# drtconway/zotmer

Measured on AMD Instinct MI355X. Metric: Gk-mers/sec kmerize k=25 on synthetic 150bp FASTQ; achieved HBM GB/s fraction, higher is better.
Workload: dtype u64

## Files before the change

zotmer_amd/csrc/context.hip:

```cpp
#include <stdarg.h>
#include <string.h>

#include "internal.hpp"
#include <vector>

namespace zk {

int fail(zk_ctx* c, int code, const char* fmt, ...) {
    char buf[512];
    va_list ap;
    va_start(ap, fmt);
    vsnprintf(buf, sizeof buf, fmt, ap);
    va_end(ap);
    if (c) c->last_error = buf;
    return code;
}

void arena_reset(zk_ctx* c) { c->arena_off = 0; }

int arena_alloc(zk_ctx* c, uint64_t bytes, void** p) {
    const uint64_t need = (bytes + 255) & ~255ull;
    if (c->arena_off + need > c->arena_size) {
        if (c->arena_off != 0)
            return fail(c, ZK_ENOMEM, "workspace too small: %llu bytes in use, %llu more needed, %llu reserved (call zk_reserve)",
// ... 254 lines not shown
    ZK_TRY(arena_alloc(c, workspace_bytes, &p));
    arena_reset(c);
    return ZK_OK;
}

int zk_release_workspace(zk_ctx* c) {
    if (!c) return ZK_EINVAL;
    enter(c);
    ZK_HIP(c, hipStreamSynchronize(c->stream));
    if (c->arena) { ZK_HIP(c, hipFree(c->arena)); c->arena = nullptr; c->arena_size = 0; c->arena_off = 0; }
    if (c->aux) { ZK_HIP(c, hipFree(c->aux)); c->aux = nullptr; c->aux_size = 0; }
    if (c->status) { ZK_HIP(c, hipFree(c->status)); c->status = nullptr; c->status_words = 0; c->epoch = 0; }
    if (c->part16) { ZK_HIP(c, hipFree(c->part16)); c->part16 = nullptr; c->part16_words = 0; }
    return ZK_OK;
}

int zk_mem_info(zk_ctx* c, uint64_t* free_bytes, uint64_t* total_bytes) {
    if (!c) return ZK_EINVAL;
    enter(c);
    size_t f = 0, t = 0;
    ZK_HIP(c, hipMemGetInfo(&f, &t));
    if (free_bytes) *free_bytes = f;
    if (total_bytes) *total_bytes = t;
    return ZK_OK;
}

int zk_tune(zk_ctx* c, int what, int value) {
    if (!c) return ZK_EINVAL;
    enter(c);
    if (what == ZK_TUNE_SORT_VARIANT) { c->sort_variant = value; return ZK_OK; }
    if (what == ZK_TUNE_PAIRS_VARIANT) { c->pairs_variant = value; return ZK_OK; }
    if (what == ZK_TUNE_SHORT_SORT) { c->short_sort = value; return ZK_OK; }
    if (what == ZK_TUNE_SIDE_DIV) { c->side_div = value; return ZK_OK; }
    if (what == ZK_TUNE_WIDE_TILES) { c->wide_tiles = value ? 1 : 0; return ZK_OK; }
    if (what == ZK_TUNE_PACKED_PAIRS) { c->packed_pairs = value ? 1 : 0; return ZK_OK; }
    if (what == ZK_TUNE_EARLY_COLLAPSE) { c->early_collapse = value < 0 ? 0 : (value > 3 ? 3 : value); return ZK_OK; }
    if (what == ZK_TUNE_COMM_SELF_LOOP) { c->comm_self_loop = value ? 1 : 0; return ZK_OK; }
    if (what == ZK_TUNE_COMM_CHUNK) { c->comm_chunk_bytes = value > 0 ? (uint64_t)value : 0; return ZK_OK; }
    if (what == ZK_TUNE_STREAM_PASS) {
#ifdef ZK_PHASES
        c->stream_pass = value < 0 ? 0 : value;
#else
        if (value < 0 || value > 3) return fail(c, ZK_EINVAL, "stream pass variant %d (0, 1, 2 or 3)", value);
        c->stream_pass = value;
#endif
        return ZK_OK;
    }
    if (what == ZK_TUNE_TAG_WORDS) { c->tag_words = value < 0 ? 0 : (value > 2 ? 2 : value); return ZK_OK; }
    if (what == ZK_TUNE_DEDUPE_VARIANT) { c->dedupe_variant = value < 0 ? -1 : (value & 3); return ZK_OK; }
    if (what == ZK_TUNE_KWAY) { c->kway = value < 0 ? 0 : (value > 2 ? 2 : value); return ZK_OK; }
    if (what == ZK_TUNE_TILE_SORT) { c->tile_sort = value ? 1 : 0; return ZK_OK; }
    if (what == ZK_TUNE_TAG_PASS) { c->tag_pass = value ? 1 : 0; return ZK_OK; }
    if (what == ZK_TUNE_DEDUPE_BITS) { c->dedupe_bits = value < 0 ? 0 : value; return ZK_OK; }
    if (what == ZK_TUNE_STRAND_BLOCKS) { c->strand_blocks = value < 0 ? 0 : (value > 5 ? 1 : value); return ZK_OK; }
    if (what == ZK_TUNE_DEDUPE_LIMIT) { c->dedupe_limit = value < 1 ? 1 : (value > 65536 ? 65536 : value); return ZK_OK; }
    if (what == ZK_TUNE_STREAM_RANGES) { c->stream_ranges = value < 0 ? 0 : (value > 4096 ? 4096 : value); return ZK_OK; }
    if (what == ZK_TUNE_XCD_GROUP) {
        if (value < 0 || value > 32 || (value & (value - 1))) return fail(c, ZK_EINVAL, "xcd group must be 0 or a power of two <= 32");
        c->xcd_group = value;
        return ZK_OK;
    }
    return fail(c, ZK_EINVAL, "unknown tuning knob %d", what);
}

int zk_debug_buffer(zk_ctx* c, void* d_buf) {
    if (!c) return ZK_EINVAL;
    enter(c);
    c->dbg = (u64*)d_buf;
    return ZK_OK;
}

int zk_profile(zk_ctx* c, int enable) {
    if (!c) return ZK_EINVAL;
    enter(c);
    ZK_HIP(c, hipStreamSynchronize(c->stream));
    for (auto& r : c->prof) { (void)hipEventDestroy(r.a); (void)hipEventDestroy(r.b); }
    c->prof.clear();
    c->profile = enable != 0;
    return ZK_OK;
}

int zk_profile_read(zk_ctx* c, int tag, uint64_t* launches, double* total_ms, uint64_t* total_bytes) {
    if (!c) return ZK_EINVAL;
    enter(c);
    ZK_HIP(c, hipStreamSynchronize(c->stream));
    uint64_t n = 0, bytes = 0;
    double ms = 0;
    for (auto& r : c->prof) {
        if (r.tag != tag) continue;
        float t = 0;
        ZK_HIP(c, hipEventElapsedTime(&t, r.a, r.b));
        n++; ms += t; bytes += r.bytes;
    }
    if (launches) *launches = n;
    if (total_ms) *total_ms = ms;
    if (total_bytes) *total_bytes = bytes;
    return ZK_OK;
}

int zk_alloc(zk_ctx* c, uint64_t bytes, void** dptr) {
    if (!c || !dptr) return ZK_EINVAL;
    enter(c);
    *dptr = nullptr;
    if (bytes == 0) bytes = 256;
    hipError_t e = hipMalloc(dptr, bytes);
    if (e != hipSuccess) return fail(c, ZK_ENOMEM, "hipMalloc(%llu) failed: %s", (unsigned long long)bytes, hipGetErrorString(e));
    return ZK_OK;
// ... 61 lines not shown
```

zotmer_amd/csrc/internal.hpp:

```cpp
#pragma once
#include <hip/hip_runtime.h>
#include <stddef.h>
#include <stdint.h>
#include <stdio.h>
#include <string>
#include <vector>

#include "../../include/zotk.h"
#include "common.hpp"

struct zk_strand_counters { u32 n_declined, fail; };
struct zk_scalars {
    u64 rle_side;
    u64 total;
    u64 acgt[4];
    u64 n_keys;
    u64 rec_info[3];
    u64 sample_n;
    u64 dedupe_flags, dedupe_n_retry, dedupe_counter, dedupe_n_big, dedupe_n_bad;
    u64 dedupe_m_cursor;
    u64 dedupe_n_in;
    u64 dedupe_n_out;
    zk_strand_counters strand;
    u64 hist_big_n;
// ... 121 lines not shown
            return zk::fail((c), ZK_EHIP, "%s failed: %s (%s:%d)", #call, hipGetErrorString(e__), __FILE__, __LINE__); \
    } while (0)
#define ZK_ARGS(c, cond) do { if (!(c)) return ZK_EINVAL; zk::enter(c); if (!(cond)) return zk::fail((c), ZK_EINVAL, "bad argument: %s", #cond); } while (0)
#define ZK_TRY(expr)             \
    do {                         \
        int r__ = (expr);        \
        if (r__ != ZK_OK) return r__; \
    } while (0)

void arena_reset(zk_ctx* c);
int arena_alloc(zk_ctx* c, uint64_t bytes, void** p);
int arena_require(zk_ctx* c, uint64_t want, uint64_t must);
int aux_require(zk_ctx* c, uint64_t bytes, char** p);
int lookback_begin(zk_ctx* c, uint64_t words, uint32_t tiles, u32* epoch, u32* ticket_base);
int part16_begin(zk_ctx* c, uint64_t words, unsigned short** out);
int check_device_error(zk_ctx* c);

void prof_begin(zk_ctx* c, int tag, uint64_t algorithmic_bytes);
void prof_end(zk_ctx* c);
void prof_add_bytes(zk_ctx* c, int tag, uint64_t bytes);

int fetch_span(zk_ctx* c, void* h_first, size_t bytes, const void* from = nullptr);
template <class T> static inline int fetch(zk_ctx* c, T* h_field, const void* from = nullptr) { return fetch_span(c, h_field, sizeof(T), from); }
int stream_sync(zk_ctx* c);

static inline uint64_t div_up(uint64_t a, uint64_t b) { return (a + b - 1) / b; }
static inline u32 grid_cap(const zk_ctx* c, uint64_t blocks, int per_cu) {
    const uint64_t mx = (uint64_t)c->num_cus * per_cu;
    return (u32)(blocks < mx ? blocks : mx);
}

constexpr int MAX_PASSES = 8;
struct PassPlan {
    int passes;
    int shift[MAX_PASSES];
    int bits[MAX_PASSES];
};
static inline PassPlan make_plan(int key_bits, int rbits, int lo = 0) {
    PassPlan p;
    if (key_bits < 1) key_bits = 1;
    if (key_bits > 64) key_bits = 64;
    p.passes = (key_bits + rbits - 1) / rbits;
    int base = key_bits / p.passes, rem = key_bits % p.passes, s = lo;
    for (int i = 0; i < MAX_PASSES; i++) { p.shift[i] = 0; p.bits[i] = 0; }
    for (int i = 0; i < p.passes; i++) {
        p.bits[i] = base + (i < rem ? 1 : 0);
        p.shift[i] = s;
        s += p.bits[i];
    }
    return p;
}
int sort_keys(zk_ctx* c, u64* keys, u64* alt, uint64_t n, int key_bits, u64** result);
int sort_pairs(zk_ctx* c, u64* keys, u64* alt, u32* vals, u32* valt, uint64_t n, int key_bits, u64** rk, u32** rv);
int sort_keys_upper(zk_ctx* c, u64* keys, u64* alt, uint64_t n, int key_bits, int lo_bit, u64** result, int prof_tag = ZK_PROF_PASS_PACKED);
int sort_pairs_upper(zk_ctx* c, u64* keys, u64* alt, u32* vals, u32* valt, uint64_t n, int key_bits, int lo_bit, u64** rk, u32** rv);
int sort_pairs_mirrored(zk_ctx* c, const u64* src_k, const u32* src_v, u64* keys, u64* alt, u32* vals, u32* valt, uint64_t n, int K,
                        u64** rk, u32** rv, int lo_bit = 0);
int sort_pairs_rbits(zk_ctx* c);
struct StreamSample { int shift; uint64_t value; double max_ratio; uint64_t seen = 0, distinct = 0; bool want_distinct = false; };
struct StreamTags { bool written = false; u64* cuts = nullptr; uint32_t blocks = 0; };
struct StreamSrc { const u8* stream; uint64_t n_bytes; int K; int mode; int lo_bit; int hi_bit = 0; StreamSample* sample = nullptr;
                   StreamTags* tags = nullptr; };
int sort_stream(zk_ctx* c, const StreamSrc& src, u64* buf_a, u64* buf_b, uint64_t cap, uint64_t* n_keys,
                uint64_t acgt[4], u64** result);
int sort_rbits(zk_ctx* c);
PassPlan sort_plan_upper(zk_ctx* c, int key_bits, int lo_bit);
int sort_first_bits(zk_ctx* c, int key_bits, int lo_bit);
constexpr int MIRROR_RBITS = 9, MIRROR_RADIX = 1 << MIRROR_RBITS;
struct MirrorHist { int passes; int shift[4]; int bits[4]; u64* raw; };
int sort_keys_upper_counted(zk_ctx* c, u64* keys, u64* alt, uint64_t n, int key_bits, int lo_bit, u64* counted, u64** result);
struct DedupeMirror { u64* out = nullptr; uint64_t cap = 0; int K = 0; };
struct DedupeResult {
    uint64_t n_out = 0;
    uint32_t flags = 0;
    uint32_t n_big = 0;
    u64 *cuts = nullptr, *nwords = nullptr, *incl = nullptr, *big = nullptr, *work = nullptr;
    u32* sub = nullptr;
    uint32_t chunks = 0;
    int pack = 0;
    int tag_bits = 0;
    bool unsorted = false;
    bool m_emitted = false;
    u64* m_words = nullptr;
    uint64_t m_cap = 0, m_placed = 0;
    MirrorHist mh = {};
    u32* retry = nullptr;
    uint32_t n_retry = 0;
};
int dedupe_pass(zk_ctx* c, const u64* keys, uint64_t n, int key_bits, int b, int pack, u64* work, uint64_t cap, DedupeResult* r,
                uint64_t* n_in = nullptr, uint64_t max_chunks = 0, const u32* tags = nullptr, const u64* tag_cuts = nullptr,
                bool unsorted = false, const DedupeMirror* mirror = nullptr);
int expand_tags(zk_ctx* c, const u32* tags, const u64* cuts, uint32_t blocks, int tag_bits, u64* keys_out, uint64_t first_block = 0, uint64_t n_blocks = 0);
int dedupe_finish(zk_ctx* c, const DedupeResult& r, u64* out_k, u32* out_c, u64* out_m = nullptr, int K = 0, int gbases = 0,
                  u64** mirror_hist = nullptr, int* mirror_group_bits = nullptr, bool packed_out = false);
int dedupe_sort_blocks(zk_ctx* c, DedupeResult& r);
int strand_blocks(zk_ctx* c, const DedupeResult& r, u64* keys_buf, uint64_t buf_words, int K, u64* out_k, u32* out_c, uint64_t cap,
                  uint64_t* n_out);
int collapse_pass(zk_ctx* c, const u64* keys, uint64_t n, int shift, int bits, int pack, u64* out, uint64_t cap, uint64_t* n_out,
                  uint64_t max_tiles = 0);
struct StreamRows { u32* rows = nullptr; u64* offs = nullptr; u32 ranges = 0, radix = 0; u32* gcodes = nullptr; u16* gvalid = nullptr;
                    u32 strands = 1;
                    bool wide = false; };
int stream_hist(zk_ctx* c, const u8* stream, uint64_t n_bytes, int K, int mode, const PassPlan& plan, u64* ghist, u32 gstride,
                u64* d_acgt, u64* d_n, u64* rec_info, u64* sample, u32 sample_cap, int sample_shift, u64 sample_value, u32* sample_n,
                void* image_room, uint64_t image_room_bytes, StreamRows* out);
struct StreamPlanes { u16* dig; int shift, bits; };
int stream_pass0(zk_ctx* c, uint64_t n_bytes, int K, int mode, int shift, int bits, const u64* ghist0, const StreamRows& rows,
                 uint64_t first_nl, bool uniform, u64* kout, uint64_t n, int variant, const StreamPlanes* planes = nullptr);
int stream_pass1(zk_ctx* c, const u32* tags, const u16* dig, uint64_t n, const u64* ghist0, uint32_t radix0, int bits1, u32* tout, u64* cuts);
int tile_sort_top_bits(uint64_t n, int key_bits, int rbits);
int tile_sort(zk_ctx* c, u64* keys, u32* vals, uint64_t n, int key_bits, int top, bool* declined);
int tile_sort_count(zk_ctx* c, const u64* keys, uint64_t n, int key_bits, int top, u64* uniq, u32* counts, uint64_t cap, uint64_t* n_unique,
                    bool* declined);
int trim(zk_ctx* c, const u64* keys, const void* cnts, int cbits, uint64_t n, u64 lo, u64 hi, u64* ok, void* oc,
         uint64_t cap, uint64_t* n_out);
int project_dedupe(zk_ctx* c, const u64* keys, uint64_t n, int shift, u64* out, uint64_t cap, uint64_t* n_out);
int subsample(zk_ctx* c, const u64* keys, uint64_t n, u64 seed, double p, u64* out, uint64_t cap, uint64_t* n_out);
int sample_pairs(zk_ctx* c, const u64* keys, const u64* cnts, uint64_t n, u64 seed, double p, u64* ok, u64* oc, uint64_t cap,
                 uint64_t* n_out);
int subsample_pairs(zk_ctx* c, u64* keys, u32* cnts, uint64_t n, u64 seed, double p, uint64_t* n_out);
int encode_list(zk_ctx* c, const u8* stream, uint64_t n_bytes, int K, int both, u64* out, uint64_t cap, uint64_t* n_out,
                uint64_t acgt[4]);
int capture_filter(zk_ctx* c, const u8* stream, uint64_t n_bytes, int K, const u64* baits, uint64_t n_baits, u8* out,
// ... 38 lines not shown
```

zotmer_amd/csrc/radix_sort.hip:

```cpp
#include <stdlib.h>
#include "internal.hpp"
#include "encode_tile.hpp"

namespace zk {

constexpr int MAX_RADIX = 1024;

enum { SRC_ARRAY = 0, SRC_STREAM = 1 };

template <int BLOCK_, int ITEMS_, int RBITS_, int ROUNDS_ = 1, int WPE_ = 1, int SEG_ = 32, bool PIPE_ = false>
struct Cfg {
    static constexpr int BLOCK = BLOCK_, ITEMS = ITEMS_, RBITS = RBITS_, ROUNDS = ROUNDS_, WPE = WPE_, SEG = SEG_;
    static constexpr bool PIPE = PIPE_;
    static_assert(SEG == 0 || (BLOCK * ITEMS < 32768 && (SEG & (SEG - 1)) == 0), "16-bit tile counts");
    static constexpr int TILE = BLOCK * ITEMS, RADIX = 1 << RBITS, NW = BLOCK / 64;
    static constexpr int EXCH = TILE / ROUNDS, IPR = ITEMS / ROUNDS;
    static_assert(ITEMS % ROUNDS == 0, "ROUNDS");
    static constexpr int DPT = (RADIX + BLOCK - 1) / BLOCK;
    static_assert(ITEMS % 2 == 0 && 2 * ITEMS < 256, "ITEMS");
    static_assert(64 * ITEMS < 65536, "per-wave ranks are 16-bit");
    static_assert(RADIX <= MAX_RADIX && RBITS * MAX_PASSES >= 64, "RBITS");
};

struct SortArgs {
// ... 580 lines not shown
                const u32 s = tid + i * BLOCK;
                if (lo + s < total && gpos[i] < a.n) a.vout[gpos[i]] = exv[s];
            }
        }
    }
#ifdef ZK_STAMPS
    asm volatile("s_waitcnt vmcnt(0)" ::: "memory");
    ZK_STAMP(7);
#endif
}

#ifdef ZK_STAMPS
#define PSTAMP(t, k) do { if (a.dbg && threadIdx.x == 0) a.dbg[(u64)(t) * 8 + (k)] = __builtin_amdgcn_s_memtime(); } while (0)
#define PSTAT(t) ((a.dbg2 && threadIdx.x == 0) ? a.dbg2 + (t) : nullptr)
#else
#define PSTAMP(t, k) do { } while (0)
#define PSTAT(t) nullptr
#endif
__device__ __forceinline__ u32 tile_of(u32 x, u32 k, u32 nx, u32 glog) {
    return ((((k >> glog) * nx) + x) << glog) | (k & ((1u << glog) - 1u));
}
__device__ __forceinline__ u32 steal_tile(const SortArgs& a, u32 x, u32 tiles) {
    for (u32 y = 1; y < a.nx; y++) {
        const u32 xx = (x + y) % a.nx;
        const u32 t = tile_of(xx, atomicAdd(a.xticket + 32 * xx, 1u), a.nx, a.glog);
        if (t < tiles) return t;
    }
    return 0xffffffffu;
}

template <class C, bool PAIRS = false>
struct PipeSmem {
    static constexpr bool IMG_FITS = sizeof(TileImage<C::TILE>) <= sizeof(u16) * C::NW * C::RADIX;
    static constexpr int IMG_WORDS = (int)(sizeof(u16) * C::NW * C::RADIX / 8);
    static constexpr int IMG_T = IMG_FITS ? (IMG_WORDS - 3) * 16 : 16;
    u64 exch[C::TILE];
    u32 exv[PAIRS ? C::TILE : 1];
    union {
        u16 cnt[C::NW][C::RADIX];
        TileImage<PipeSmem::IMG_T> img;
    };
    u32 digit_off[C::RADIX];
    u64 gbase[C::RADIX];
    u32 wsum[C::NW];
    u32 ticket;
    u32 total_live;
    u32 abort;
};

template <class C, int SRC, int VAR = 0>
__global__ __launch_bounds__(C::BLOCK, C::WPE) void pass_pipe_kernel(SortArgs a, u32 tiles) {
    constexpr int BLOCK = C::BLOCK, ITEMS = C::ITEMS, RADIX = C::RADIX, NW = C::NW, DPT = C::DPT, TILE = C::TILE;
    constexpr bool PAIRS = VAR == 5 || VAR == 6;
    constexpr bool ATOM = VAR == 3 || VAR == 4 || VAR == 6, TAGS = VAR == 2 || VAR == 3;
    static_assert(!PAIRS || SRC == SRC_ARRAY, "pairs come from arrays");
    static_assert(!ATOM || (SRC == SRC_ARRAY && NW >= 2), "the counters of the adds are the first two rows of the per-wave counters");
    static_assert(C::ROUNDS == 1, "the pipeline parks a whole tile in LDS");
    constexpr int NS = RADIX / 64;
    __shared__ PipeSmem<C, VAR == 5 || VAR == 6> sm;
    static_assert(SRC == SRC_ARRAY || PipeSmem<C>::IMG_FITS, "the tile image lives in the counter area");
    static_assert(SRC == SRC_ARRAY || (ITEMS == 16 && PipeSmem<C>::IMG_WORDS <= 2 * BLOCK), "stream source: 16 consecutive windows per thread");
    const int tid = threadIdx.x, lane = tid & 63, wave = __builtin_amdgcn_readfirstlane(tid >> 6);
    const u32 dmask = (1u << a.bits) - 1u;
    u16* mycnt = sm.cnt[wave];

    if (tid == 0) sm.abort = 0;
    u32* cnt32 = reinterpret_cast<u32*>(&sm.cnt[0][0]);
    if (ATOM && tid < RADIX) cnt32[tid] = 0;
    bool dirty = false;
    const u32 first = take_ticket(a.ticket, &sm.ticket) - a.ticket_base;
    if (first < (u32)NS) {
        constexpr int U = 32;
        __builtin_amdgcn_s_setprio(3);
        u64* carry = sm.exch;
        if (tid < 64) carry[tid] = 0;
        __syncthreads();
        const u64 tag = st_pack(ZK_ST_INCLUSIVE, a.epoch, 0);
        const u32 batches = (tiles + U - 1) / U;
        for (u32 b = (u32)wave; b < batches; b += NW) {
            const u32 t0 = b * U;
            const u32 nt = (tiles - t0 < (u32)U) ? tiles - t0 : (u32)U;
            __amdgpu_buffer_rsrc_t rs = __builtin_amdgcn_make_buffer_rsrc((void*)(a.part + (u64)t0 * RADIX + (u64)first * 64), 0, 0x7fffffff, 0x00020000);
            __amdgpu_buffer_rsrc_t rd = __builtin_amdgcn_make_buffer_rsrc((void*)(a.status + (u64)t0 * RADIX + (u64)first * 64), 0, 0x7fffffff, 0x00020000);
            u16 x[U];
#pragma unroll
            for (int k = 0; k < U; k++)
                x[k] = ((u32)k < nt) ? (u16)__builtin_amdgcn_raw_buffer_load_b16(rs, 2 * lane, k * RADIX * 2, 16) : (u16)0x8000u;
            for (int spins = 0;; spins++) {
                u32 all = 0x8000u;
#pragma unroll
                for (int k = 0; k < U; k++) all &= x[k];
                if (all & 0x8000u) break;
                if (spins > ZK_SPIN_LIMIT) { atomicOr(a.err, ZK_DERR_SPIN_TIMEOUT | (8u << 8)); break; }
                __builtin_amdgcn_s_sleep(2);
#pragma unroll
                for (int k = 0; k < U; k++)
                    if (!(x[k] & 0x8000u)) x[k] = (u16)__builtin_amdgcn_raw_buffer_load_b16(rs, 2 * lane, k * RADIX * 2, 16);
            }
            u32 sum = 0;
#pragma unroll
            for (int k = 0; k < U; k++) {
                x[k] &= 0x7fffu;
                sum += x[k];
            }
            volatile u64* cw = carry + lane;
            u64 cv = *cw;
            int spins = 0;
// ... 417 lines not shown

    static int begin_pass(zk_ctx* c, SortArgs& a, u32 tiles, u32 tickets, bool pipe, bool stamps = true) {
        const bool seg = !pipe && C::SEG > 0;
        ZK_TRY(lookback_begin(c, seg ? ((uint64_t)tiles / (C::SEG > 0 ? C::SEG : 1) + 2) * C::RADIX : (uint64_t)tiles * C::RADIX, tickets,
                              &a.epoch, &a.ticket_base));
        if (pipe || seg) ZK_TRY(part16_begin(c, (uint64_t)tiles * C::RADIX, &a.part));
        a.status = c->status;
        a.ticket = c->d_ticket;
        a.err = c->d_err;
        a.dbg = stamps ? c->dbg : nullptr;
        a.dbg2 = (stamps && c->dbg) ? c->dbg + 8ull * tiles : nullptr;
        return ZK_OK;
    }
    template <bool PAIRS>
    static int begin_pipe(zk_ctx* c, SortArgs& a, u32 tiles, u32* grid, bool stamps) {
        u32 g = (u32)c->num_cus * (sizeof(PipeSmem<C, PAIRS>) > 80 * 1024 ? 1 : 2);
        if (g > tiles) g = tiles;
        g += C::RADIX / 64;
        ZK_TRY(begin_pass(c, a, tiles, g, true, stamps));
        ZK_HIP(c, hipMemsetAsync(c->d_xticket, 0, 8 * 32 * sizeof(u32), c->stream));
        a.xticket = c->d_xticket;
        a.nx = 1u;
        a.glog = 0;
        *grid = g;
        return ZK_OK;
    }

    template <int SRC, bool PAIRS>
    static int launch_pass(zk_ctx* c, SortArgs a) {
        const u32 tiles = tiles_for(a, SRC);
        if (tiles == 0) return ZK_OK;
        ZK_TRY(begin_pass(c, a, tiles, tiles, false));
        prof_begin(c, SRC == SRC_STREAM ? ZK_PROF_PASS_STREAM : (PAIRS ? ZK_PROF_PASS_PAIRS : ZK_PROF_PASS_KEYS),
                   SRC == SRC_STREAM ? a.n_bytes + 8 * a.n : (PAIRS ? 24 : 16) * a.n);
        hipLaunchKernelGGL((pass_kernel<C, SRC, PAIRS>), dim3(tiles), dim3(C::BLOCK), 0, c->stream, a);
        prof_end(c);
        ZK_HIP(c, hipGetLastError());
        return ZK_OK;
    }

    template <int SRC>
    static int launch_pipe(zk_ctx* c, SortArgs a) {
      if constexpr (C::PIPE) {
        const u32 tiles = tiles_for(a, SRC);
        if (tiles == 0) return ZK_OK;
        u32 grid;
        ZK_TRY(begin_pipe<false>(c, a, tiles, &grid, true));
        a.nx = (c->xcd_group > 0 && c->num_xcd == 8) ? 8u : 1u;
        while ((1 << (a.glog + 1)) <= c->xcd_group) a.glog++;
        prof_begin(c, SRC == SRC_STREAM ? ZK_PROF_PASS_STREAM : (a.prof_tag ? a.prof_tag : ZK_PROF_PASS_KEYS),
                   SRC == SRC_STREAM ? a.n_bytes + 8 * a.n : (a.tags_out ? 12 : 16) * a.n);
        if (SRC == SRC_ARRAY && a.tags_out && a.straddle)
            hipLaunchKernelGGL((pass_pipe_kernel<C, SRC_ARRAY, 3>), dim3(grid), dim3(C::BLOCK), 0, c->stream, a, tiles);
        else if (SRC == SRC_ARRAY && a.straddle)
            hipLaunchKernelGGL((pass_pipe_kernel<C, SRC_ARRAY, 4>), dim3(grid), dim3(C::BLOCK), 0, c->stream, a, tiles);
        else if (SRC == SRC_ARRAY && a.tags_out)
            hipLaunchKernelGGL((pass_pipe_kernel<C, SRC_ARRAY, 2>), dim3(grid), dim3(C::BLOCK), 0, c->stream, a, tiles);
        else if (SRC == SRC_ARRAY && a.prof_tag == ZK_PROF_PASS_PACKED)
            hipLaunchKernelGGL((pass_pipe_kernel<C, SRC, 1>), dim3(grid), dim3(C::BLOCK), 0, c->stream, a, tiles);
        else
            hipLaunchKernelGGL((pass_pipe_kernel<C, SRC, 0>), dim3(grid), dim3(C::BLOCK), 0, c->stream, a, tiles);
        prof_end(c);
        ZK_HIP(c, hipGetLastError());
      }
      return ZK_OK;
    }
    static constexpr bool PIPE_PAIRS = C::PIPE && C::ITEMS <= 8;
    static int launch_pipe_pairs(zk_ctx* c, SortArgs a) {
      if constexpr (PIPE_PAIRS) {
        const u32 tiles = (u32)div_up(a.n, C::TILE);
        if (tiles == 0) return ZK_OK;
        u32 grid;
        ZK_TRY(begin_pipe<true>(c, a, tiles, &grid, false));
        prof_begin(c, ZK_PROF_PASS_PAIRS, 24 * a.n);
        if (a.straddle) hipLaunchKernelGGL((pass_pipe_kernel<C, SRC_ARRAY, 6>), dim3(grid), dim3(C::BLOCK), 0, c->stream, a, tiles);
        else hipLaunchKernelGGL((pass_pipe_kernel<C, SRC_ARRAY, 5>), dim3(grid), dim3(C::BLOCK), 0, c->stream, a, tiles);
        prof_end(c);
        ZK_HIP(c, hipGetLastError());
      }
      return ZK_OK;
    }
    static constexpr bool WIDE = C::PIPE && C::RBITS == 9 && C::BLOCK == 512;
    static u32 keys_pass_tile(zk_ctx* c) { return (WIDE && c->wide_tiles) ? 16384u : (u32)C::TILE; }
    static int launch_keys_pass(zk_ctx* c, const SortArgs& a) {
        if (WIDE && c->wide_tiles) return launch_wide_pass(c, a);
        if (C::PIPE) return launch_pipe<SRC_ARRAY>(c, a);
        return launch_pass<SRC_ARRAY, false>(c, a);
    }

    template <int SRC>
    static int launch_hist(zk_ctx* c, const SortArgs& src, const PassPlan& plan, u64* ghist, u64* acgt, u64* d_n,
                           u64* sample = nullptr, u32 sample_cap = 0, int sample_shift = 0, u64 sample_value = 0) {
        HistArgs h;
        h.sample = sample; h.sample_cap = sample_cap; h.sample_shift = sample_shift; h.sample_value = sample_value;
        h.sample_n = (u32*)&c->d_scalars->sample_n;
        if (sample) ZK_HIP(c, hipMemsetAsync(h.sample_n, 0, sizeof(u64), c->stream));
        h.src = src;
        h.plan = plan;
        h.ghist = ghist;
        h.acgt = acgt;
        h.tiles = tiles_for(src, SRC);
        h.rec_info = nullptr;
        ZK_HIP(c, hipMemsetAsync(ghist, 0, sizeof(u64) * MAX_PASSES * C::RADIX, c->stream));
        if (SRC == SRC_STREAM && src.n_bytes) {
            h.rec_info = c->d_scalars->rec_info;
            ZK_HIP(c, hipMemsetAsync(h.rec_info, 0, 3 * sizeof(u64), c->stream));
            hipLaunchKernelGGL(first_newline_kernel, dim3(1), dim3(256), 0, c->stream, src.stream, (u64)src.n_bytes, h.rec_info);
        }
        if (acgt) ZK_HIP(c, hipMemsetAsync(acgt, 0, sizeof(u64) * 4, c->stream));
        u32 grid = grid_cap(c, h.tiles, 8);
        if (grid == 0) grid = 1;
        prof_begin(c, SRC == SRC_STREAM ? ZK_PROF_HIST_STREAM : ZK_PROF_HIST_ARRAY, SRC == SRC_STREAM ? src.n_bytes : 8 * src.n);
        if constexpr (SRC == SRC_STREAM && C::ITEMS == 16 && C::BLOCK <= 512) {
            if (src.mode != ZK_KEYS_BOTH) hipLaunchKernelGGL((hist_kernel<C, SRC, true>), dim3(grid), dim3(C::BLOCK), 0, c->stream, h);
            else hipLaunchKernelGGL((hist_kernel<C, SRC, false>), dim3(grid), dim3(C::BLOCK), 0, c->stream, h);
        } else {
            hipLaunchKernelGGL((hist_kernel<C, SRC, false>), dim3(grid), dim3(C::BLOCK), 0, c->stream, h);
        }
        prof_end(c);
        ZK_HIP(c, hipGetLastError());
        hipLaunchKernelGGL(hist_scan_kernel, dim3(1), dim3(256), 0, c->stream, ghist, plan.passes, (int)C::RADIX, d_n);
        ZK_HIP(c, hipGetLastError());
        return ZK_OK;
    }

    static int sort_keys(zk_ctx* c, u64* keys, u64* alt, uint64_t n, int key_bits, u64** result, int lo_bit = 0, int prof_tag = 0,
                         u64* counted = nullptr) {
        PassPlan plan = make_plan(key_bits - lo_bit, C::RBITS, lo_bit);
        u64* ghist = counted;
        if (!counted) ZK_TRY(arena_alloc(c, sizeof(u64) * MAX_PASSES * C::RADIX, (void**)&ghist));
        SortArgs a = {};
        a.kin = keys; a.n = n;
        a.prof_tag = prof_tag;
        if (counted) {
            hipLaunchKernelGGL(hist_scan_kernel, dim3(1), dim3(256), 0, c->stream, ghist, plan.passes, (int)C::RADIX, &c->d_scalars->n_keys);
            ZK_HIP(c, hipGetLastError());
        } else {
            ZK_TRY(launch_hist<SRC_ARRAY>(c, a, plan, ghist, nullptr, &c->d_scalars->n_keys));
        }
        u64* in = keys; u64* out = alt;
        for (int p = 0; p < plan.passes; p++) {
            a.kin = in; a.kout = out; a.shift = plan.shift[p]; a.bits = plan.bits[p];
            a.ghist = ghist + p * C::RADIX;
            ZK_TRY(launch_keys_pass(c, a));
            u64* t = in; in = out; out = t;
        }
        *result = in;
        return ZK_OK;
    }

    static int sort_pairs(zk_ctx* c, u64* keys, u64* alt, u32* vals, u32* valt, uint64_t n, int key_bits, u64** rk, u32** rv,
                          const u64* src_k = nullptr, const u32* src_v = nullptr, int mirror_K = 0, int lo_bit = 0, bool unordered = false) {
        PassPlan plan = make_plan(key_bits - lo_bit, C::RBITS, lo_bit);
        u64* ghist;
        ZK_TRY(arena_alloc(c, sizeof(u64) * MAX_PASSES * C::RADIX, (void**)&ghist));
        SortArgs a = {};
        a.kin = mirror_K ? src_k : keys; a.n = n; a.mirror_K = mirror_K;
        ZK_TRY(launch_hist<SRC_ARRAY>(c, a, plan, ghist, nullptr, &c->d_scalars->n_keys));
        const u64* in = mirror_K ? src_k : keys; const u32* vi = mirror_K ? src_v : vals;
        u64* out = mirror_K ? keys : alt; u32* vo = mirror_K ? vals : valt;
        for (int p = 0; p < plan.passes; p++) {
            a.kin = in; a.kout = out; a.vin = vi; a.vout = vo; a.shift = plan.shift[p]; a.bits = plan.bits[p];
            a.ghist = ghist + p * C::RADIX;
            a.mirror_K = (p == 0) ? mirror_K : 0;
            if constexpr (PIPE_PAIRS) {
                a.straddle = nullptr;
                if (unordered && p <= 1)
                    ZK_TRY(straddle_bitmap(c, n, (u32)C::TILE, p == 1 ? ghist : nullptr, 1u << plan.bits[0], (u32)C::RADIX, &a.straddle));
                ZK_TRY(launch_pipe_pairs(c, a));
            } else
            ZK_TRY((launch_pass<SRC_ARRAY, true>(c, a)));
            in = out; vi = vo;
            out = (out == keys) ? alt : keys;
            vo = (vo == vals) ? valt : vals;
        }
        *rk = const_cast<u64*>(in); *rv = const_cast<u32*>(vi);
        return ZK_OK;
    }

    static int stream_count(zk_ctx* c, const StreamSrc& src, const StreamPlan& sp, const SortArgs& a, u64* ghist, u64* buf_b, uint64_t cap,
                            StreamRows* srows, uint64_t* n, uint64_t acgt[4]) {
        u64* d_acgt = c->d_scalars->acgt;
        u64* d_n = &c->d_scalars->n_keys;
        u64* sample = sp.sampling ? buf_b : nullptr;
        const int sample_shift = sp.sampling ? src.sample->shift : 0;
        const u64 sample_value = sp.sampling ? src.sample->value : 0;
        if (sp.ranged) {
            u64* rec_info = c->d_scalars->rec_info;
            ZK_HIP(c, hipMemsetAsync(rec_info, 0, ZK_SPAN(rec_info, sample_n), c->stream));
            hipLaunchKernelGGL(first_newline_kernel, dim3(1), dim3(256), 0, c->stream, src.stream, (u64)src.n_bytes, rec_info);
            ZK_TRY(stream_hist(c, src.stream, src.n_bytes, src.K, src.mode, sp.plan, ghist, (u32)C::RADIX, d_acgt, d_n, rec_info,
                               sample, SAMPLE_CAP, sample_shift, sample_value, (u32*)&c->d_scalars->sample_n,
                               (char*)buf_b + (sp.sampling ? 24ull * SAMPLE_CAP : 0), 8 * cap - (sp.sampling ? 24ull * SAMPLE_CAP : 0), srows));
            hipLaunchKernelGGL(hist_scan_kernel, dim3(1), dim3(256), 0, c->stream, ghist, sp.plan.passes, (int)C::RADIX, d_n);
            ZK_HIP(c, hipGetLastError());
        } else {
// ... 142 lines not shown
typedef Cfg<1024, 8, 9, 1, 4, 32, true> V7;
static_assert(V3::RBITS == MIRROR_RBITS && V3::RADIX == MIRROR_RADIX, "dedupe_finish counts the digits of the default geometry");
int launch_wide_pass(zk_ctx* c, const SortArgs& a) { return Sorter<V6>::launch_pipe<SRC_ARRAY>(c, a); }
#define ZK_SORT_CASES(CALL)                         \
        case 0: return Sorter<V0>::CALL;            \
        case 1: return Sorter<V1>::CALL;            \
        case 2: return Sorter<V2>::CALL;            \
        case 4: return Sorter<V4>::CALL;            \
        case 5: return Sorter<V5>::CALL;            \
        case 6: return Sorter<V6>::CALL;            \
        default: return Sorter<V3>::CALL;
#define ZK_SORT_DISPATCH(c, CALL) switch ((c)->sort_variant) { ZK_SORT_CASES(CALL) }
#define ZK_PAIRS_DISPATCH(c, CALL) switch ((c)->pairs_variant) { case 7: return Sorter<V7>::CALL; ZK_SORT_CASES(CALL) }

static int sort_keys_lsd(zk_ctx* c, u64* keys, u64* alt, uint64_t n, int key_bits, u64** result) {
    ZK_SORT_DISPATCH(c, sort_keys(c, keys, alt, n, key_bits, result));
}
static int sort_pairs_lsd(zk_ctx* c, u64* keys, u64* alt, u32* vals, u32* valt, uint64_t n, int key_bits, u64** rk, u32** rv) {
    ZK_PAIRS_DISPATCH(c, sort_pairs(c, keys, alt, vals, valt, n, key_bits, rk, rv));
}

int sort_keys(zk_ctx* c, u64* keys, u64* alt, uint64_t n, int key_bits, u64** result) {
    *result = keys;
    if (n == 0) return ZK_OK;
    const int top = c->tile_sort ? tile_sort_top_bits(n, key_bits, sort_rbits(c)) : 0;
    if (top) {
        u64* res = nullptr;
        bool declined = false;
        ZK_TRY(sort_keys_upper(c, keys, alt, n, key_bits, key_bits - top, &res, ZK_PROF_PASS_KEYS));
        ZK_TRY(tile_sort(c, res, nullptr, n, key_bits, top, &declined));
        *result = res;
        if (!declined) return ZK_OK;
        return sort_keys_lsd(c, res, res == keys ? alt : keys, n, key_bits, result);
    }
    return sort_keys_lsd(c, keys, alt, n, key_bits, result);
}

int sort_pairs(zk_ctx* c, u64* keys, u64* alt, u32* vals, u32* valt, uint64_t n, int key_bits, u64** rk, u32** rv) {
    *rk = keys; *rv = vals;
    if (n == 0) return ZK_OK;
    const int top = c->tile_sort ? tile_sort_top_bits(n, key_bits, sort_pairs_rbits(c)) : 0;
    if (top) {
        u64* k1 = nullptr; u32* v1 = nullptr;
        bool declined = false;
        ZK_TRY(sort_pairs_upper(c, keys, alt, vals, valt, n, key_bits, key_bits - top, &k1, &v1));
        ZK_TRY(tile_sort(c, k1, v1, n, key_bits, top, &declined));
        *rk = k1; *rv = v1;
        if (!declined) return ZK_OK;
        return sort_pairs_lsd(c, k1, k1 == keys ? alt : keys, v1, v1 == vals ? valt : vals, n, key_bits, rk, rv);
    }
    return sort_pairs_lsd(c, keys, alt, vals, valt, n, key_bits, rk, rv);
}

int sort_keys_upper(zk_ctx* c, u64* keys, u64* alt, uint64_t n, int key_bits, int lo_bit, u64** result, int prof_tag) {
    *result = keys;
    if (n == 0 || lo_bit >= key_bits) return ZK_OK;
    ZK_SORT_DISPATCH(c, sort_keys(c, keys, alt, n, key_bits, result, lo_bit, prof_tag));
}

int sort_keys_upper_counted(zk_ctx* c, u64* keys, u64* alt, uint64_t n, int key_bits, int lo_bit, u64* counted, u64** result) {
    *result = keys;
    if (n == 0 || lo_bit >= key_bits) return ZK_OK;
    return Sorter<V3>::sort_keys(c, keys, alt, n, key_bits, result, lo_bit, ZK_PROF_PASS_PACKED, counted);
}

int sort_pairs_upper(zk_ctx* c, u64* keys, u64* alt, u32* vals, u32* valt, uint64_t n, int key_bits, int lo_bit, u64** rk, u32** rv) {
    *rk = keys; *rv = vals;
    if (n == 0) return ZK_OK;
    ZK_PAIRS_DISPATCH(c, sort_pairs(c, keys, alt, vals, valt, n, key_bits, rk, rv, nullptr, nullptr, 0, lo_bit));
}

int sort_pairs_mirrored(zk_ctx* c, const u64* src_k, const u32* src_v, u64* keys, u64* alt, u32* vals, u32* valt, uint64_t n, int K,
                        u64** rk, u32** rv, int lo_bit) {
    *rk = keys; *rv = vals;
    if (n == 0) return ZK_OK;
    ZK_PAIRS_DISPATCH(c, sort_pairs(c, keys, alt, vals, valt, n, 2 * K, rk, rv, src_k, src_v, K, lo_bit, true));
}

int sort_rbits(zk_ctx* c) { ZK_SORT_DISPATCH(c, rbits()); }
int sort_pairs_rbits(zk_ctx* c) { ZK_PAIRS_DISPATCH(c, rbits()); }

PassPlan sort_plan_upper(zk_ctx* c, int key_bits, int lo_bit) { return make_plan(key_bits - lo_bit, sort_rbits(c), lo_bit); }

int sort_first_bits(zk_ctx* c, int key_bits, int lo_bit) {
    if (lo_bit >= key_bits) return 0;
    return make_plan(key_bits - lo_bit, sort_rbits(c), lo_bit).bits[0];
}

int sort_stream(zk_ctx* c, const StreamSrc& src, u64* buf_a, u64* buf_b, uint64_t cap, uint64_t* n_keys,
                uint64_t acgt[4], u64** result) {
    *result = buf_a;
    *n_keys = 0;
    if (acgt) acgt[0] = acgt[1] = acgt[2] = acgt[3] = 0;
    if (src.n_bytes == 0) return ZK_OK;
    if ((uintptr_t)src.stream & 15) return fail(c, ZK_EINVAL, "base stream must be 16-byte aligned");
    ZK_SORT_DISPATCH(c, sort_stream(c, src, buf_a, buf_b, cap, n_keys, acgt, result));
}

}
```

zotmer_amd/csrc/strand_blocks.hip:

```cpp
#include "tile_group.hpp"

namespace zk {

constexpr int SB_ITEMS = 16, SB_GROUPS = 2048;
constexpr u32 SB_GROUP_MAX = 128;
typedef TileSortSmem<SB_ITEMS, SB_GROUPS, false> StrandSmem;
constexpr int SB_BLOCK_BITS = 18;

__global__ __launch_bounds__(256) void strand_mirror_kernel(const u64* __restrict__ in, const u64* __restrict__ cuts, const u64* __restrict__ incl,
                                                            const u64* __restrict__ nwords, u32 chunks, int pack, int K, u64* __restrict__ out_m,
                                                            MirrorHist mh, const u32* __restrict__ list, u64* cursor, u64 m_cap) {
    __shared__ u32 bins[4 * 512];
    __shared__ u64 placed;
    const bool hist = mh.passes > 0;
    if (hist) {
        for (int q = threadIdx.x; q < 4 * 512; q += blockDim.x) bins[q] = 0;
        __syncthreads();
    }
    const u64 maxc = (1ull << pack) - 1;
    for (u32 t = blockIdx.x; t < chunks; t += gridDim.x) {
        const u32 v = list ? list[t] : t;
        const u64 cnt = nwords[v];
        u64 dst0 = incl[v] - cnt;
        if (list) {
// ... 251 lines not shown
    *n_out = 0;
    const uint64_t uc = r.n_out;
    if (uc == 0) return ZK_OK;
    if (!(K & 1) || r.n_big || r.chunks != (1u << SB_BLOCK_BITS)) return fail(c, ZK_EINTERNAL, "strand_blocks: K %d, %u big counts, %u blocks", K, r.n_big, r.chunks);
    const uint64_t a8w = ((8 * uc + 255) & ~255ull) / 8;
    if (2 * a8w > buf_words) return fail(c, ZK_EINTERNAL, "strand_blocks: %llu words do not fit twice in %llu", (unsigned long long)uc, (unsigned long long)buf_words);
    if (2 * uc > cap) return fail(c, ZK_ENOSPC, "output holds %llu entries, the table has %llu", (unsigned long long)cap, (unsigned long long)(2 * uc));
    const int pk = r.pack, key_bits = 2 * K + pk, lo_bit = key_bits - SB_BLOCK_BITS;
    u64* mw = keys_buf;
    u64* malt = keys_buf + a8w;
    MirrorHist mh = {};
    bool fused = r.m_emitted && r.m_words >= keys_buf && r.m_words + r.m_cap <= keys_buf + buf_words && uc <= r.m_cap && c->sort_variant == 3;
    if (fused) {
        const PassPlan plan = sort_plan_upper(c, key_bits, lo_bit);
        fused = plan.passes == r.mh.passes;
        for (int p = 0; fused && p < plan.passes; p++) fused = plan.shift[p] == r.mh.shift[p] && plan.bits[p] == r.mh.bits[p];
        const uint64_t before = (uint64_t)(r.m_words - keys_buf), behind = buf_words - before;
        if (before < a8w && behind < 2 * a8w) fused = false;
        if (fused) malt = before >= a8w ? keys_buf : r.m_words + a8w;
    }
    if (fused) {
        mw = r.m_words;
        mh = r.mh;
        uint64_t placed = r.m_placed;
        prof_begin(c, ZK_PROF_SELECT, 16 * uc);
        if (r.n_retry) {
            hipLaunchKernelGGL(strand_mirror_kernel, dim3(grid_cap(c, r.n_retry, 8)), dim3(256), 0, c->stream, r.work, r.cuts, r.incl, r.nwords, r.n_retry, pk, K,
                               mw, mh, r.retry, &c->d_scalars->dedupe_m_cursor, (u64)r.m_cap);
        }
        prof_end(c);
        if (r.n_retry) {
            ZK_HIP(c, hipGetLastError());
            ZK_TRY(fetch(c, &c->h_scalars->dedupe_m_cursor));
            ZK_TRY(stream_sync(c));
            placed = c->h_scalars->dedupe_m_cursor;
        }
        if (placed != uc) return fail(c, ZK_EINTERNAL, "strand_blocks: %llu mirror words for %llu entries", (unsigned long long)placed, (unsigned long long)uc);
    } else {
        if (c->sort_variant == 3) {
            const PassPlan plan = sort_plan_upper(c, key_bits, lo_bit);
            if (plan.passes <= 4) {
                ZK_TRY(arena_alloc(c, sizeof(u64) * MAX_PASSES * 512, (void**)&mh.raw));
                ZK_HIP(c, hipMemsetAsync(mh.raw, 0, sizeof(u64) * MAX_PASSES * 512, c->stream));
                mh.passes = plan.passes;
                for (int p = 0; p < plan.passes; p++) { mh.shift[p] = plan.shift[p]; mh.bits[p] = plan.bits[p]; }
            }
        }
        prof_begin(c, ZK_PROF_SELECT, 16 * uc);
        hipLaunchKernelGGL(strand_mirror_kernel, dim3((u32)c->num_cus * 8), dim3(256), 0, c->stream, r.work, r.cuts, r.incl, r.nwords, r.chunks, pk, K, mw, mh,
                           (const u32*)nullptr, (u64*)nullptr, (u64)0);
        prof_end(c);
        ZK_HIP(c, hipGetLastError());
    }
    u64* sk = nullptr;
    if (mh.passes) ZK_TRY(sort_keys_upper_counted(c, mw, malt, uc, key_bits, lo_bit, mh.raw, &sk));
    else ZK_TRY(sort_keys_upper(c, mw, malt, uc, key_bits, lo_bit, &sk));
    u64* mstart;
    u32* declined;
    ZK_TRY(arena_alloc(c, sizeof(u64) * ((1ull << SB_BLOCK_BITS) + 1), (void**)&mstart));
    ZK_TRY(arena_alloc(c, sizeof(u32) * r.chunks, (void**)&declined));
    StrandArgs a = {};
    a.cw = r.work; a.cuts = r.cuts; a.nwords = r.nwords; a.incl = r.incl; a.m = sk; a.mstart = mstart;
    a.ok = out_k; a.oc = out_c; a.pack = pk; a.pshift = lo_bit;
    a.n_declined = &c->d_scalars->strand.n_declined;
    a.declined = declined;
    u32* fail = &c->d_scalars->strand.fail;
    prof_begin(c, ZK_PROF_UNION, 8 * 2 * uc + 12 * 2 * uc);
    hipLaunchKernelGGL(strand_starts_kernel, dim3(((1u << SB_BLOCK_BITS) + 256) / 256), dim3(256), 0, c->stream, sk, (u64)uc, lo_bit, mstart);
    ZK_HIP(c, hipMemsetAsync(&c->d_scalars->strand, 0, sizeof(zk_strand_counters), c->stream));
    hipLaunchKernelGGL(strand_block_union_kernel, dim3(r.chunks), dim3(TS_BLOCK), 0, c->stream, a);
    prof_end(c);
    ZK_HIP(c, hipGetLastError());
    ZK_TRY(fetch(c, &c->h_scalars->strand));
    ZK_TRY(check_device_error(c));
    const uint32_t n_declined = c->h_scalars->strand.n_declined;
    bool other_way = n_declined && c->strand_blocks == 3;
    if (n_declined && !other_way) {
        const uint32_t grid = n_declined < 2u * (uint32_t)c->num_cus ? n_declined : 2u * (uint32_t)c->num_cus;
        u64* scratch;
        ZK_TRY(arena_alloc(c, sizeof(u64) * StrandSmem::CAP * grid, (void**)&scratch));
        prof_begin(c, ZK_PROF_UNION, 0);
        hipLaunchKernelGGL(strand_big_block_kernel, dim3(grid), dim3(TS_BLOCK), 0, c->stream, a, n_declined, scratch, fail);
        prof_end(c);
        ZK_HIP(c, hipGetLastError());
        ZK_TRY(fetch(c, &c->h_scalars->strand));
        ZK_TRY(check_device_error(c));
        other_way = c->h_scalars->strand.fail != 0;
    }
    if (!other_way) {
        *n_out = 2 * uc;
        return ZK_OK;
    }
    DedupeResult rs = r;
    ZK_TRY(dedupe_sort_blocks(c, rs));
    char* aux;
    ZK_TRY(aux_require(c, 8 * a8w, &aux));
    ZK_TRY(dedupe_finish(c, rs, (u64*)aux, nullptr, nullptr, K, 0, nullptr, nullptr, true));
    u64* ms = nullptr;
    ZK_TRY(sort_keys_upper(c, sk, sk == mw ? malt : mw, uc, key_bits, pk, &ms));
    return union_sum_packed_ab(c, (const u64*)aux, uc, ms, uc, pk, out_k, out_c, cap, n_out, true);
}

}
```

Baseline: 176.1.

## Add unordered strand-block mirror sort using straddle-bitmap atomic scatter passes

Adds a strand_blocks=6 mode in which the mirror-word sort runs its first two radix passes with a straddle bitmap and a new pipe-kernel variant that uses atomic scatter. Within-bucket order is not kept, which drops the ordered tile-to-tile lookback for those passes. It costs extra bitmap construction and only fits consumers that can tolerate unordered ties. It is active only when the tuning knob is set to 6.

```diff
diff --git a/zotmer_amd/csrc/context.hip b/zotmer_amd/csrc/context.hip
--- a/zotmer_amd/csrc/context.hip
+++ b/zotmer_amd/csrc/context.hip
@@ -330,7 +330,7 @@
     if (what == ZK_TUNE_TILE_SORT) { c->tile_sort = value ? 1 : 0; return ZK_OK; }
     if (what == ZK_TUNE_TAG_PASS) { c->tag_pass = value ? 1 : 0; return ZK_OK; }
     if (what == ZK_TUNE_DEDUPE_BITS) { c->dedupe_bits = value < 0 ? 0 : value; return ZK_OK; }
-    if (what == ZK_TUNE_STRAND_BLOCKS) { c->strand_blocks = value < 0 ? 0 : (value > 5 ? 1 : value); return ZK_OK; }
+    if (what == ZK_TUNE_STRAND_BLOCKS) { c->strand_blocks = value < 0 ? 0 : (value > 6 ? 1 : value); return ZK_OK; }
     if (what == ZK_TUNE_DEDUPE_LIMIT) { c->dedupe_limit = value < 1 ? 1 : (value > 65536 ? 65536 : value); return ZK_OK; }
     if (what == ZK_TUNE_STREAM_RANGES) { c->stream_ranges = value < 0 ? 0 : (value > 4096 ? 4096 : value); return ZK_OK; }
     if (what == ZK_TUNE_XCD_GROUP) {
diff --git a/zotmer_amd/csrc/internal.hpp b/zotmer_amd/csrc/internal.hpp
--- a/zotmer_amd/csrc/internal.hpp
+++ b/zotmer_amd/csrc/internal.hpp
@@ -197,7 +197,8 @@
 }
 int sort_keys(zk_ctx* c, u64* keys, u64* alt, uint64_t n, int key_bits, u64** result);
 int sort_pairs(zk_ctx* c, u64* keys, u64* alt, u32* vals, u32* valt, uint64_t n, int key_bits, u64** rk, u32** rv);
-int sort_keys_upper(zk_ctx* c, u64* keys, u64* alt, uint64_t n, int key_bits, int lo_bit, u64** result, int prof_tag = ZK_PROF_PASS_PACKED);
+int sort_keys_upper(zk_ctx* c, u64* keys, u64* alt, uint64_t n, int key_bits, int lo_bit, u64** result, int prof_tag = ZK_PROF_PASS_PACKED,
+                    bool unordered = false);
 int sort_pairs_upper(zk_ctx* c, u64* keys, u64* alt, u32* vals, u32* valt, uint64_t n, int key_bits, int lo_bit, u64** rk, u32** rv);
 int sort_pairs_mirrored(zk_ctx* c, const u64* src_k, const u32* src_v, u64* keys, u64* alt, u32* vals, u32* valt, uint64_t n, int K,
                         u64** rk, u32** rv, int lo_bit = 0);
@@ -213,7 +214,8 @@
 int sort_first_bits(zk_ctx* c, int key_bits, int lo_bit);
 constexpr int MIRROR_RBITS = 9, MIRROR_RADIX = 1 << MIRROR_RBITS;
 struct MirrorHist { int passes; int shift[4]; int bits[4]; u64* raw; };
-int sort_keys_upper_counted(zk_ctx* c, u64* keys, u64* alt, uint64_t n, int key_bits, int lo_bit, u64* counted, u64** result);
+int sort_keys_upper_counted(zk_ctx* c, u64* keys, u64* alt, uint64_t n, int key_bits, int lo_bit, u64* counted, u64** result,
+                            bool unordered = false);
 struct DedupeMirror { u64* out = nullptr; uint64_t cap = 0; int K = 0; };
 struct DedupeResult {
     uint64_t n_out = 0;
diff --git a/zotmer_amd/csrc/radix_sort.hip b/zotmer_amd/csrc/radix_sort.hip
--- a/zotmer_amd/csrc/radix_sort.hip
+++ b/zotmer_amd/csrc/radix_sort.hip
@@ -656,7 +656,7 @@
 __global__ __launch_bounds__(C::BLOCK, C::WPE) void pass_pipe_kernel(SortArgs a, u32 tiles) {
     constexpr int BLOCK = C::BLOCK, ITEMS = C::ITEMS, RADIX = C::RADIX, NW = C::NW, DPT = C::DPT, TILE = C::TILE;
     constexpr bool PAIRS = VAR == 5 || VAR == 6;
-    constexpr bool ATOM = VAR == 3 || VAR == 4 || VAR == 6, TAGS = VAR == 2 || VAR == 3;
+    constexpr bool ATOM = VAR == 3 || VAR == 4 || VAR == 6 || VAR == 7, TAGS = VAR == 2 || VAR == 3;
     static_assert(!PAIRS || SRC == SRC_ARRAY, "pairs come from arrays");
     static_assert(!ATOM || (SRC == SRC_ARRAY && NW >= 2), "the counters of the adds are the first two rows of the per-wave counters");
     static_assert(C::ROUNDS == 1, "the pipeline parks a whole tile in LDS");
@@ -1180,6 +1180,8 @@
                    SRC == SRC_STREAM ? a.n_bytes + 8 * a.n : (a.tags_out ? 12 : 16) * a.n);
         if (SRC == SRC_ARRAY && a.tags_out && a.straddle)
             hipLaunchKernelGGL((pass_pipe_kernel<C, SRC_ARRAY, 3>), dim3(grid), dim3(C::BLOCK), 0, c->stream, a, tiles);
+        else if (SRC == SRC_ARRAY && a.straddle && a.prof_tag == ZK_PROF_PASS_PACKED)
+            hipLaunchKernelGGL((pass_pipe_kernel<C, SRC_ARRAY, 7>), dim3(grid), dim3(C::BLOCK), 0, c->stream, a, tiles);
         else if (SRC == SRC_ARRAY && a.straddle)
             hipLaunchKernelGGL((pass_pipe_kernel<C, SRC_ARRAY, 4>), dim3(grid), dim3(C::BLOCK), 0, c->stream, a, tiles);
         else if (SRC == SRC_ARRAY && a.tags_out)
@@ -1253,7 +1255,7 @@
     }
 
     static int sort_keys(zk_ctx* c, u64* keys, u64* alt, uint64_t n, int key_bits, u64** result, int lo_bit = 0, int prof_tag = 0,
-                         u64* counted = nullptr) {
+                         u64* counted = nullptr, bool unordered = false) {
         PassPlan plan = make_plan(key_bits - lo_bit, C::RBITS, lo_bit);
         u64* ghist = counted;
         if (!counted) ZK_TRY(arena_alloc(c, sizeof(u64) * MAX_PASSES * C::RADIX, (void**)&ghist));
@@ -1270,6 +1272,11 @@
         for (int p = 0; p < plan.passes; p++) {
             a.kin = in; a.kout = out; a.shift = plan.shift[p]; a.bits = plan.bits[p];
             a.ghist = ghist + p * C::RADIX;
+            if constexpr (C::PIPE) {
+                a.straddle = nullptr;
+                if (unordered && p <= 1)
+                    ZK_TRY(straddle_bitmap(c, n, keys_pass_tile(c), p == 1 ? ghist : nullptr, 1u << plan.bits[0], (u32)C::RADIX, &a.straddle));
+            }
             ZK_TRY(launch_keys_pass(c, a));
             u64* t = in; in = out; out = t;
         }
@@ -1518,16 +1525,16 @@
     return sort_pairs_lsd(c, keys, alt, vals, valt, n, key_bits, rk, rv);
 }
 
-int sort_keys_upper(zk_ctx* c, u64* keys, u64* alt, uint64_t n, int key_bits, int lo_bit, u64** result, int prof_tag) {
+int sort_keys_upper(zk_ctx* c, u64* keys, u64* alt, uint64_t n, int key_bits, int lo_bit, u64** result, int prof_tag, bool unordered) {
     *result = keys;
     if (n == 0 || lo_bit >= key_bits) return ZK_OK;
-    ZK_SORT_DISPATCH(c, sort_keys(c, keys, alt, n, key_bits, result, lo_bit, prof_tag));
-}
-
-int sort_keys_upper_counted(zk_ctx* c, u64* keys, u64* alt, uint64_t n, int key_bits, int lo_bit, u64* counted, u64** result) {
+    ZK_SORT_DISPATCH(c, sort_keys(c, keys, alt, n, key_bits, result, lo_bit, prof_tag, nullptr, unordered));
+}
+
+int sort_keys_upper_counted(zk_ctx* c, u64* keys, u64* alt, uint64_t n, int key_bits, int lo_bit, u64* counted, u64** result, bool unordered) {
     *result = keys;
     if (n == 0 || lo_bit >= key_bits) return ZK_OK;
-    return Sorter<V3>::sort_keys(c, keys, alt, n, key_bits, result, lo_bit, ZK_PROF_PASS_PACKED, counted);
+    return Sorter<V3>::sort_keys(c, keys, alt, n, key_bits, result, lo_bit, ZK_PROF_PASS_PACKED, counted, unordered);
 }
 
 int sort_pairs_upper(zk_ctx* c, u64* keys, u64* alt, u32* vals, u32* valt, uint64_t n, int key_bits, int lo_bit, u64** rk, u32** rv) {
diff --git a/zotmer_amd/csrc/strand_blocks.hip b/zotmer_amd/csrc/strand_blocks.hip
--- a/zotmer_amd/csrc/strand_blocks.hip
+++ b/zotmer_amd/csrc/strand_blocks.hip
@@ -327,9 +327,10 @@
         prof_end(c);
         ZK_HIP(c, hipGetLastError());
     }
+    const bool unordered = c->strand_blocks == 6;
     u64* sk = nullptr;
-    if (mh.passes) ZK_TRY(sort_keys_upper_counted(c, mw, malt, uc, key_bits, lo_bit, mh.raw, &sk));
-    else ZK_TRY(sort_keys_upper(c, mw, malt, uc, key_bits, lo_bit, &sk));
+    if (mh.passes) ZK_TRY(sort_keys_upper_counted(c, mw, malt, uc, key_bits, lo_bit, mh.raw, &sk, unordered));
+    else ZK_TRY(sort_keys_upper(c, mw, malt, uc, key_bits, lo_bit, &sk, ZK_PROF_PASS_PACKED, unordered));
     u64* mstart;
     u32* declined;
     ZK_TRY(arena_alloc(c, sizeof(u64) * ((1ull << SB_BLOCK_BITS) + 1), (void**)&mstart));
```

After: 173.8. 0.987x the previous value.
